# baldhat/yolov10-3D

Measured on AMD Instinct MI355X. Metric: train_images_per_sec, higher is better.
Workload: dtype bf16

## Files before the change

include/y3d.h:

```cpp
#ifndef Y3D_H
#define Y3D_H
#include <stdint.h>

#ifdef __cplusplus
extern "C" {
#endif

enum { Y3D_F32 = 0, Y3D_BF16 = 1 };
enum { Y3D_OK = 0, Y3D_ERR_INVALID = -1, Y3D_ERR_HIP = -2 };

const char* y3d_last_error(void);
int y3d_abi_version(void);
int y3d_device_info(char* name, int name_len, int* compute_units, int* lds_bytes, int* clock_khz);

int y3d_pack_weight_fwd(int dtype, const float* w_oihw, void* out, int Cout, int Cin_g, int Cin_g_pad, int kh, int kw, void* stream);
int y3d_pack_weight_dgrad(int dtype, const float* w_oihw, void* out, int Cout, int Cin_g, int groups, int kh, int kw, void* stream);
int y3d_mt_pack_weights(int dtype, const int64_t* desc, const int* chunk_tensor, const int* chunk_off, int nchunks, int chunk, void* stream);
int y3d_mt_fp8w_quantize(const int64_t* desc, const int* row_begin, int ntensors, int nrows, void* stream);
int y3d_fp8w_dequantize(const uint8_t* codes, const float* scale, float* w, int rows, int K, void* stream);
int y3d_fp8_quantize_act(const void* x, int64_t xsw, int64_t M, int C, uint8_t* q, uint8_t* s, void* stream);
int y3d_fp8_pack_weight_fwd(const uint8_t* codes, const float* scale, int rows, int Cg, uint8_t* wq, uint8_t* ws, void* stream);
int y3d_conv3x3_fp8_ok(int B, int H, int W, int Cin, int Cout, int groups);
int y3d_conv3x3_fp8_stat_rows(int B, int H, int W);
int y3d_fp8_scale_pitch(int C);
int y3d_conv3x3_fp8_fwd(const uint8_t* xq, const uint8_t* xs, int B, int H, int W, int Cin, const uint8_t* wq, const uint8_t* ws, void* y, int64_t ysw,
                        int Cout, int groups, float* stat_partials, const float* scale, const float* shift, int act, void* stream);
int y3d_fp8_quantize_grad(const void* dy, int64_t sw, const float* scale, int64_t M, int C, uint8_t* q, uint8_t* s, void* stream);
int y3d_fp8_pack_weight_dgrad(const uint8_t* codes, int Cout, int Cin, int groups, int lo, int hi, uint8_t* wq, uint8_t* ws, void* stream);
int y3d_conv3x3_fp8_dgrad_ok(int B, int H, int W, int Cin, int Cout, int groups);
int y3d_conv3x3_fp8_dgrad(const uint8_t* dyq, const uint8_t* dys, int64_t qsw, int spitch, int lo, int hi, int B, int H, int W, const uint8_t* wq, const uint8_t* ws,
                          void* dx, int64_t dxsw, int Cin, int groups, void* stream);
int y3d_conv_kpad(int dtype, int k_total);
int y3d_conv_stat_blocks(int B, int Ho, int Wo);
int y3d_conv2d_stat_rows(int dtype, int B, int H, int W, int Cin, int Cout, int groups, int kh, int kw, int stride, int pad);
enum { Y3D_OP_FWD = 0, Y3D_OP_BWD_DATA = 1, Y3D_OP_BWD_WEIGHT = 2 };
enum { Y3D_EPI_RAW = 0, Y3D_EPI_PARTIALS = 1, Y3D_EPI_AFFINE = 2, Y3D_EPI_AFFINE_RES = 3, Y3D_EPI_BIAS = 4 };
enum {
  Y3D_ROUTE_GENERIC = 0,
  Y3D_ROUTE_STREAM1X1 = 1,
  Y3D_ROUTE_SMALL = 2,
  Y3D_ROUTE_SMALL_S2 = 3,
  Y3D_ROUTE_S2_DGRAD = 4,
  Y3D_ROUTE_TILE8 = 5,
  Y3D_ROUTE_TILE16 = 6,
  Y3D_ROUTE_WIDE3_8 = 7,
  Y3D_ROUTE_WIDE3_16 = 8,
  Y3D_ROUTE_FLAT = 9,
  Y3D_ROUTE_WGRAD_SMALL = 10,
  Y3D_ROUTE_WGRAD_TILE = 11,
  Y3D_ROUTE_WGRAD_STREAM1X1 = 12
};
int y3d_conv2d_route(int dtype, int op, int epi, int B, int H, int W, int Cin, int Cout, int groups, int kh, int kw, int stride, int pad);
int y3d_conv2d_fwd(int dtype, const void* x, int64_t xsb, int64_t xsh, int64_t xsw, int B, int H, int W, int Cin,
                   const void* w_packed, const float* bias, void* y, int64_t ysw, int Ho, int Wo, int Cout, int groups,
                   int kh, int kw, int stride, int pad, float* stat_partials, void* stream);
int y3d_conv2d_fwd_affine(int dtype, const void* x, int64_t xsb, int64_t xsh, int64_t xsw, int B, int H, int W, int Cin,
                          const void* w_packed, const float* scale, const float* shift, int act, void* y, int64_t ysw, int Ho, int Wo,
                          int Cout, int groups, int kh, int kw, int stride, int pad, void* stream);
int y3d_conv2d_fwd_affine_res_ok(int dtype, int B, int H, int W, int Cin, int Cout, int groups, int kh, int kw, int stride, int pad);
int y3d_conv2d_fwd_affine_res(int dtype, const void* x, int64_t xsb, int64_t xsh, int64_t xsw, int B, int H, int W, int Cin,
                              const void* w_packed, const float* scale, const float* shift, int act, const void* res, int64_t rsw, void* y,
                              int64_t ysw, int Ho, int Wo, int Cout, int groups, int kh, int kw, int stride, int pad, void* stream);
int y3d_conv2d_bwd_data(int dtype, const void* dy, int64_t dsb, int64_t dsh, int64_t dsw, int B, int Ho, int Wo, int Cout,
                        const void* w_packed_dgrad, void* dx, int64_t xsw, int H, int W, int Cin, int groups, int kh, int kw,
                        int stride, int pad, void* stream);
int y3d_conv2d_wgrad_splits(int dtype, int B, int Ho, int Wo, int Cout, int Cin_g, int groups, int kh, int kw);
int y3d_conv2d_wgrad_plan(int dtype, int B, int H, int W, int Cin, int Cout, int groups, int kh, int kw, int stride, int pad);
int y3d_set_tile_kernels(int enable);
int y3d_set_stream1x1(int enable);
int y3d_get_stream1x1(void);
int y3d_get_tile_kernels(void);
int y3d_set_bn_wide_slabs(int enable);
int y3d_conv2d_bwd_weight(int dtype, const void* x, int64_t xsb, int64_t xsh, int64_t xsw, int B, int H, int W, int Cin,
                          int Cin_real, const void* dy, int64_t dsw, int Ho, int Wo, int Cout, int groups, int kh, int kw,
                          int stride, int pad, float* slab, int nsplit, float* grad_oihw, int accumulate, void* stream);

int y3d_dw_blocks(int64_t M);
int y3d_dw_wgrad_blocks(int64_t M);
int y3d_dw_pack_weight(const float* w_oihw, float* out_taps_c, int C, int kh, int kw, void* stream);
int y3d_dwconv2d_fwd(int dtype, const void* x, int64_t xsb, int64_t xsh, int64_t xsw, int B, int H, int W, int C,
                     const float* w_packed, void* y, int64_t ysw, int Ho, int Wo, int kh, int kw, int stride, int pad,
                     float* stat_partials, void* stream);
int y3d_dwconv2d_fwd_affine(int dtype, const void* x, int64_t xsb, int64_t xsh, int64_t xsw, int B, int H, int W, int C,
                            const float* w_packed, const float* scale, const float* shift, int act, int res_mode, const void* res, int64_t rsw,
                            void* z, int64_t zsw, int Ho, int Wo, int kh, int kw, int stride, int pad, void* stream);
int y3d_dwconv2d_bwd_data(int dtype, const void* dy, int64_t dsb, int64_t dsh, int64_t dsw, int B, int Ho, int Wo, int C,
                          const float* w_packed, void* dx, int64_t xsw, int H, int W, int kh, int kw, int stride, int pad,
                          void* stream);
int y3d_dwconv2d_bwd_weight(int dtype, const void* x, int64_t xsb, int64_t xsh, int64_t xsw, int B, int H, int W, int C,
                            const void* dy, int64_t dsw, int Ho, int Wo, int kh, int kw, int stride, int pad, float* slab,
                            float* grad_oihw, int accumulate, void* stream);

int y3d_bn_finalize(const float* partials, int nblk, int C, int64_t count, const float* gamma, const float* beta, float eps,
                    float momentum, float* running_mean, float* running_var, float* mean, float* invstd, float* scale,
                    float* shift, void* stream);
int y3d_bn_eval_scale(int C, const float* gamma, const float* beta, const float* running_mean, const float* running_var,
                      float eps, float* scale, float* shift, void* stream);
int y3d_bn_act_fwd(int dtype, const void* y, int64_t ysw, const float* scale, const float* shift, int act, int res_mode,
                   const void* res, int64_t rsw, void* z, int64_t zsw, int64_t P, int C, void* stream);
int y3d_bn_act_fwd_q(const void* y, int64_t ysw, const float* scale, const float* shift, int act, void* z, int64_t zsw, uint8_t* q, uint8_t* s,
                     int64_t P, int C, void* stream);
int y3d_bn_bwd_blocks(int64_t P, int C);
int y3d_bn_act_bwd_reduce(int dtype, const void* y, int64_t ysw, const void* dz, int64_t dsw, const void* res, int64_t rsw,
                          const float* scale, const float* shift, const float* mean, const float* invstd, int act,
                          int res_mode, float* partials, int64_t P, int C, void* stream);
int y3d_bn_bwd_finalize(const float* partials, int nblk, int C, int64_t count, float* dgamma, float* dbeta, int accumulate,
                        float* mean_g, float* mean_gx, void* stream);
int y3d_bn_act_bwd_apply(int dtype, const void* y, int64_t ysw, const void* dz, int64_t dsw, const void* res, int64_t rsw,
                         const float* scale, const float* shift, const float* mean, const float* invstd,
                         const float* mean_g, const float* mean_gx, int act, int res_mode, int train, void* dy, int64_t dysw,
                         void* dres, int64_t drsw, int64_t P, int C, void* stream);
int y3d_colsum_partials(int dtype, const void* x, int64_t xsw, float* partials, int64_t P, int C, void* stream);

int y3d_maxpool_fwd(int dtype, const void* x, int64_t xsb, int64_t xsh, int64_t xsw, void* y, int64_t ysw, uint8_t* argmax,
                    int B, int H, int W, int C, int k, void* stream);
int y3d_maxpool_bwd(int dtype, const void* dy, int64_t dsw, const uint8_t* argmax, void* dx, int64_t xsw, int B, int H, int W,
                    int C, int k, void* stream);
int y3d_upsample2x_fwd(int dtype, const void* x, int64_t xsb, int64_t xsh, int64_t xsw, void* y, int64_t ysw, int B, int H, int W,
                       int C, void* stream);
int y3d_upsample2x_bwd(int dtype, const void* dy, int64_t dsb, int64_t dsh, int64_t dsw, void* dx, int64_t xsw, int B, int H,
                       int W, int C, void* stream);
int y3d_copy2d(int dtype, const void* x, int64_t xsw, void* y, int64_t ysw, int64_t P, int C, void* stream);
int y3d_occupy_cus(int n, const int* flag, float* buf, int64_t nbuf, void* stream);
int y3d_add2d(int dtype, const void* a, int64_t asw, const void* b, int64_t bsw, void* y, int64_t ysw, int64_t P, int C, void* stream);
int y3d_nchw_to_nhwc(int dtype, const float* x_nchw, void* y_nhwc, int B, int C, int H, int W, int Cpad, void* stream);
int y3d_stem_im2col(int dtype, const float* x_nchw, void* out, int B, int H, int W, int Ho, int Wo, void* stream);
int y3d_stem_im2col_u8(int dtype, const uint8_t* x, int hwc, void* out, int B, int H, int W, int Ho, int Wo, void* stream);
int y3d_stem_conv_eval(const void* x, int in_mode, const float* wcol, const float* scale, const float* shift, int act, void* y, int64_t ysw,
                       int B, int H, int W, int Cout, void* stream);
int y3d_stem_conv_train_rows(int B, int H, int W);
int y3d_stem_conv_train(const void* x, int in_mode, const float* wcol, void* y, int64_t ysw, void* xcol, float* part, int B, int H, int W,
                        int Cout, void* stream);
int y3d_nhwc_to_nchw(int dtype, const void* x_nhwc, int64_t xsw, float* y_nchw, int B, int C, int H, int W, void* stream);
int y3d_proj_fwd(int dtype, const void* x, int64_t xsw, const float* w, const float* bias, void* y, int64_t ysw, int64_t P,
                 int Cin, int Cout, void* stream);
int y3d_proj_bwd_data(int dtype, const void* dy, int64_t dsw, const float* w, void* dx, int64_t xsw, int64_t P, int Cin, int Cout,
                      void* stream);
int y3d_proj_blocks(int64_t P);
int y3d_proj_bwd_weight(int dtype, const void* x, int64_t xsw, const void* dy, int64_t dsw, float* slab, float* bias_slab,
                        float* grad_w, float* grad_b, int accumulate, int64_t P, int Cin, int Cout, void* stream);
int y3d_slab_reduce(const float* slab, float* out, int nblk, int64_t n, int accumulate, void* stream);
int y3d_proj_group_fwd(int dtype, int nb, int cin, const void* x, int64_t xsw, const int* xoff, const float* const* w,
                       const float* const* b, const int* couts, void* y, int64_t ysw, int64_t P, void* stream);
int y3d_proj_group_bwd_data(int dtype, int nb, int cin, const void* dy, int64_t dsw, const int* xoff, const float* const* w,
                            const int* couts, void* dx, int64_t xsw, int64_t P, void* stream);
int y3d_proj_group_fwd_bn_mfma(int nb, int cin, const void* y_pre, int64_t ysw, const int* xoff, const float* const* w, const float* const* b,
                               const int* couts, const float* scale, const float* shift, int act, void* out, int64_t osw, int64_t P,
                               void* stream);
int y3d_proj_group_bwd_weight_bn_mfma_blocks(int64_t P);
int y3d_proj_group_bwd_weight_bn_mfma(int nb, int cin, const void* y_pre, int64_t ysw, const int* xoff, const void* dout, int64_t dsw,
                                      const int* couts, const float* scale, const float* shift, int act, float* slab, float* bslab,
                                      float* const* dw, float* const* db, int64_t P, void* stream);
int y3d_proj_group_bn_bwd_blocks(int64_t P);
int y3d_proj_group_bn_bwd(int mode, int nb, int cin, const void* y_pre, int64_t ysw, const int* xoff, const void* dout, int64_t dsw,
                          const float* const* w, const int* couts, const float* scale, const float* shift, const float* mean,
                          const float* invstd, const float* mean_g, const float* mean_gx, int act, float* partials, int nblk, void* dy,
                          int64_t dysw, int64_t P, int C, void* stream);
int y3d_proj_group_blocks(int64_t P);
int y3d_proj_group_fwd_bn(int dtype, int nb, int cin, const void* y_pre, int64_t xsw, const int* xoff, const float* const* w,
                          const float* const* b, const int* couts, const float* scale, const float* shift, int act, void* out,
                          int64_t ysw, int64_t P, void* stream);
int y3d_proj_group_bwd_weight_bn(int dtype, int nb, int cin, const void* y_pre, int64_t xsw, const int* xoff, const void* dy, int64_t dsw,
                                 const int* couts, const float* scale, const float* shift, int act, float* slab, float* bslab,
                                 float* const* dw, float* const* db, int64_t P, void* stream);
int y3d_proj_group_bwd_weight(int dtype, int nb, int cin, const void* x, int64_t xsw, const int* xoff, const void* dy, int64_t dsw,
                              const int* couts, float* slab, float* bslab, float* const* dw, float* const* db, int64_t P, void* stream);

int y3d_attn_fwd(int dtype, const void* qkv, int64_t qsw, void* out, int64_t osw, float* lse, int B, int N, int nh, int kd, int hd,
                 float scale, void* stream);
int y3d_attn_bwd(int dtype, const void* qkv, int64_t qsw, const void* out, int64_t osw, const void* dout, int64_t dsw,
                 const void* dv_extra, int64_t esw, const float* lse, float* delta, void* dqkv, int64_t gsw, int B, int N, int nh,
                 int kd, int hd, float scale, void* stream);

int y3d_tal3d_scratch_floats(int B, int n, int A, int topk);
int y3d_pad_targets(const float* rows, int nbox, int width, int B, int cap, float scale_x, float scale_y, float* out, int* n_used,
                    void* stream);
int y3d_tal3d_assign(int dtype, int nl, const void* const* maps, const int64_t* psw, const int* H, const int* W, const float* strides,
                     int B, int nc, const float* gt, int n, const float* calib, const float* mean_sizes, int topk, float alpha,
                     float beta, float gamma, int mode, float* scratch, uint8_t* fg_mask, int* target_gt_idx, float* target_scores, float* scal,
                     const int* n_used, void* stream);
int y3d_loss3d(int dtype, int nl, const void* const* maps, const int64_t* psw, void* const* grads, const int64_t* gsw, const int* H,
               const int* W, const float* strides, int B, int nc, const float* gt, int n, const uint8_t* fg_mask,
               const int* target_gt_idx, const float* target_scores, const float* scal, float w_loss2d, float w_cls, float w_depth,
               float w_offset3d, float w_size3d, float w_heading, float grad_scale, float* partials, float* items, void* stream);

int y3d_distill_loss(int dtype, int nl, const void* const* embs, const int64_t* psw, const int* H, const int* W, int B, int C,
                     const void* teacher, int teacher_dtype, int th, int tw, int64_t tsb, int64_t tsc, int64_t tsh, int64_t tsw,
                     const float* gt, int n, const uint8_t* fg_mask, const int* target_gt_idx, const float* scal, const uint8_t* mixed,
                     int img_w, int img_h, float T, float weight, int criterion, int no_mixup, int cap, int* counts, int* idx,
                     void* rows, float* partials, float* loss, void* stream);
int y3d_distill_scatter(int dtype, const void* rows, const int* idx, const int* nrows, const float* scale, int cap, int C, void* grad,
                        int64_t sb, int64_t sh, int64_t sw, int a0, int H, int W, void* stream);

int y3d_tal2d_assign(int dtype, int nl, const void* const* maps, const int64_t* psw, const int* H, const int* W, const float* strides,
                     int B, int nc, const float* gt, int n, int topk, float alpha, float beta, float* scratch, uint8_t* fg_mask,
                     int* target_gt_idx, float* target_scores, float* scal, const int* n_used, void* stream);
int y3d_loss2d(int dtype, int nl, const void* const* maps, const int64_t* psw, void* const* grads, const int64_t* gsw, const int* H,
               const int* W, const float* strides, int B, int nc, const float* gt, int n, const uint8_t* fg_mask,
               const int* target_gt_idx, const float* target_scores, const float* scal, float w_box, float w_cls, float w_dfl,
               float grad_scale, float* partials, float* items, void* stream);
int y3d_tal2d_scratch_floats(int B, int n, int A, int topk);
int y3d_tal2d_assign_crowded(int dtype, int nl, const void* const* maps, const int64_t* psw, const int* H, const int* W, const float* strides,
                             int B, int nc, const float* gt, int n, int topk, float alpha, float beta, float* scratch, uint8_t* fg_mask,
                             int* target_gt_idx, float* target_scores, float* scal, const int* n_used, void* stream);

int y3d_topk_cells(int dtype, const void* cls, int64_t psw, int B, int HW, int nc, int K, int* out_idx, void* stream);
int y3d_patch_gather(int dtype, const void* x, int64_t xsb, int64_t xsh, int64_t xsw, const int* idx, void* out, int B, int H, int W,
                     int C, int K, int ps, void* stream);
int y3d_head3d_scatter(int dtype, const void* cls, int64_t csw, const void* reg, int64_t rsw, const int* idx, void* map, int B, int HW,
                       int nc, int no, int K, void* stream);
int y3d_head3d_decode(int dtype, int nl, const void* const* maps, const int* H, const int* W, const float* strides, int B, int nc,
                      float* y, void* stream);
int y3d_head2d_decode(int dtype, int nl, const void* const* maps, const int* H, const int* W, const float* strides, int B, int nc,
                      float* y, void* stream);
int y3d_v10_postprocess_scratch_floats(int B, int A, int nc, int max_det);
int y3d_v10_postprocess(const float* y, int B, int C, int A, int nc, int max_det, int boxes_first, float* reg, float* scores,
                        int64_t* labels, float* scratch, void* stream);

int y3d_kitti_image_aug(const unsigned char* const* src, const unsigned char* const* src2, const int* hw, const int* flip, const double* trans_inv,
                        int B, int out_h, int out_w, int mode, void* out, void* stream);
int y3d_kde_depth_fusion(const float* predsO, int B, int K, const float* predsM, int KM, int C, float thres, float iou_thres, int nprop,
                         float* out, void* stream);
int y3d_kitti_decode(const float* preds, int B, int K, const double* calib, const double* ratio, const double* inv_trans,
                     const double* mean_size, int nc, int use_camera_dis, double threshold, double* out, unsigned char* keep, void* stream);
int y3d_kitti_encode_labels(const double* rec, const int* img_i, const double* img_f, int B, int out_w, int out_h, double min_depth,
                            double max_depth, int use_camera_dis, const double* mean_size, int n_cls, int max_objs, int64_t* cls,
                            double* bboxes, float* center_2d, float* size_2d, double* center_3d, double* size_3d, double* depth,
                            int64_t* heading_bin, double* heading_res, float* batch_idx, int* counts, double* calib, double* ratio_pad,
                            void* stream);
int y3d_json3d_encode_labels(const double* rec, const int* img_i, const double* img_f, int B, int dataset, int out_w, int out_h,
                             double min_depth, double max_depth, int use_camera_dis, const double* mean_size, int n_cls, int max_objs,
                             int64_t* cls, double* bboxes, float* center_2d, float* size_2d, double* center_3d, double* size_3d,
                             double* depth, int64_t* heading_bin, double* heading_res, float* batch_idx, int* counts, double* calib,
                             double* ratio_pad, void* stream);
int y3d_yolo2d_image_aug(const unsigned char* const* src, int n_src, const int* rec_i, const double* rec_f, const unsigned char* lut, int B,
                         int imgsz, int mode, void* out, void* stream);
int y3d_yolo2d_encode_labels(const float* rec, int n_rec, const int* lab_i, const float* lab_f, int B, int imgsz, int cap, float* cls,
                             float* bboxes, float* batch_idx, int* counts, void* stream);
int y3d_letterbox_image(const unsigned char* const* src_table, int n_src, const int* rec, int B, int H, int W, int mode, void* out,
                        void* stream);
int y3d_letterbox_labels(const float* rec, int n_rec, const int* lab_i, const float* lab_f, int B, int H, int W, int cap, float* cls,
                         float* bboxes, float* batch_idx, int* counts, void* stream);
int y3d_predict_rows(const float* preds, const float* meta, float conf, const int* classes, int n_cls, int B, int K, float* out, int* counts,
                     void* stream);
int y3d_predict3d_rows(const float* preds, int B, int K, const double* calib, const double* P2, const double* ratio,
                       const double* inv_trans, const double* mean_size, int nc, int use_camera_dis, double conf, const int* classes,
                       int n_cls, double* rows, double* corners3d, double* corners_img, int* counts, void* stream);

int y3d_kitti_eval_max_boxes(void);
int y3d_kitti_box_overlaps(int metric, const float* gt, const float* dt, const int* gt_off, const int* dt_off, const int64_t* ov_off,
                           int n_img, float* out, void* stream);
int y3d_kitti_eval_thresholds(const float* gt, const int* gt_code, const float* dt, const int* dt_code, const int* gt_off, const int* dt_off,
                              const int64_t* ov_off, const float* ov, int n_img, int total_gt, int metric, const int* cd, int ncd,
                              const double* min_ov, int nk, float* tp_score, int* nvalid, void* stream);
int y3d_kitti_eval_counts(const float* gt, const int* gt_code, const float* dt, const int* dt_code, const int* gt_off, const int* dt_off,
                          const int64_t* ov_off, const float* ov, int n_img, int metric, const int* cd, int ncd, const double* min_ov, int nk,
                          const float* thr, const int* nthr, int compute_aos, int* cnt, double* sim, double* pr, void* stream);

int y3d_det_metrics_max_gts(void);
int y3d_det_metrics_max_dets(void);
int y3d_box_iou(const float* box1, int n1, const float* box2, int n2, float eps, float* out, void* stream);
int y3d_match_predictions(const float* iou, const int* gt_cls, int n_gt, const int* det_cls, int n_det, const float* thr, int n_thr,
                          int* tp, void* stream);
int y3d_box_match_batch(int mode, const void* preds, const unsigned char* keep, int B, int K, const double* meta, int img_h, int img_w,
                        int single_cls, const float* gt_img, const float* gt_cls, const float* gt_box, int n_gt, const float* thr,
                        int n_thr, int* tp, double* conf, int* cls, int* status, void* stream);
int y3d_confusion_batch(int mode, const void* preds, const unsigned char* keep, int B, int K, const double* meta, int img_h, int img_w,
                        int single_cls, const float* gt_img, const float* gt_cls, const float* gt_box, int n_gt, int nc, double conf,
                        double iou_thres, int* matrix, int* status, void* stream);
int y3d_confusion_image(const float* gt_box, const int* gt_cls, int n_gt, const void* det, int det_f64, int n_det, int nc, double conf,
                        double iou_thres, int* matrix, int* status, void* stream);
int y3d_ap_per_class(const int* tp, const double* conf, const int* cls, int64_t n, const int* ucls, const double* nl, int nc, int n_thr,
                     const double* x_ap, int n_ap, const double* x_curve, int n_curve, double* ap, double* p_curve, double* r_curve,
                     void* stream);

int y3d_mt_sqnorm(const int64_t* grad_ptrs, const int64_t* sizes, const int* chunk_tensor, const int* chunk_off, int nchunks, int chunk,
                  float* partials, void* stream);
int y3d_mt_copy(const int64_t* src_ptrs, const int64_t* dst_ptrs, const int64_t* sizes, const int* chunk_tensor, const int* chunk_off,
                int nchunks, int chunk, float scale, void* stream);
int y3d_mt_clip_coef(const float* partials, int nchunks, float max_norm, float* out_norm_clip, void* stream);
int y3d_mt_sgd(const int64_t* param_ptrs, const int64_t* grad_ptrs, const int64_t* buf_ptrs, const int64_t* sizes, const float* lr,
               const float* wd, const int* chunk_tensor, const int* chunk_off, int nchunks, int chunk, float momentum, int nesterov,
               int first_step, const float* norm_clip, void* stream);

int y3d_mt_adamw(const int64_t* param_ptrs, const int64_t* grad_ptrs, const int64_t* m_ptrs, const int64_t* v_ptrs, const int64_t* sizes,
                 const float* lr, const float* wd, const int* chunk_tensor, const int* chunk_off, int nchunks, int chunk, float beta1, float beta2,
                 float eps, float bias_corr1, float bias_corr2_sqrt, const float* norm_clip, void* stream);
int y3d_mt_ema(const int64_t* ema_ptrs, const int64_t* model_ptrs, const int64_t* sizes, const int* reps, const int* chunk_tensor,
               const int* chunk_off, int nchunks, int chunk, float decay, float one_minus_decay, const float* guard, void* stream);

#ifdef __cplusplus
}
#endif
#endif
```

yolov10-3d_amd/_lib.py:

```python
from __future__ import annotations

import ctypes
import os
import re

_HERE = os.path.dirname(os.path.abspath(__file__))
LIB_PATH = os.path.join(_HERE, "liby3d_hip.so")
HEADER = os.path.join(os.path.dirname(_HERE), "include", "y3d.h")

F32, BF16 = 0, 1

_CT = {"int": ctypes.c_int, "int64_t": ctypes.c_int64, "float": ctypes.c_float, "double": ctypes.c_double}


class Y3DError(RuntimeError):
    pass


def parse_header(path: str = HEADER):
    src = open(path).read()
    src = re.sub(r"/\*.*?\*/", " ", src, flags=re.S)
    protos = {}
    for m in re.finditer(r"(const\s+char\s*\*|int)\s+(y3d_\w+)\s*\(([^;{]*?)\)\s*;", src, flags=re.S):
        ret, name, args = m.group(1), m.group(2), m.group(3).strip()
        argtypes = []
        if args and args != "void":
            for a in args.split(","):
                a = a.strip()
                if "*" in a:
                    argtypes.append(ctypes.c_void_p)
                else:
                    toks = a.split()
                    t = toks[1] if toks[0] == "const" else toks[0]
                    argtypes.append(_CT[t])
        protos[name] = (ctypes.c_char_p if "char" in ret else ctypes.c_int, argtypes)
    return protos


_PLAIN_INT = {"abi_version", "conv_kpad", "conv_stat_blocks", "conv2d_stat_rows", "conv2d_route", "conv2d_wgrad_splits", "conv2d_wgrad_plan", "set_tile_kernels", "set_stream1x1", "set_bn_wide_slabs", "get_stream1x1", "get_tile_kernels", "dw_blocks", "dw_wgrad_blocks", "bn_bwd_blocks", "proj_blocks", "proj_group_blocks", "proj_group_bn_bwd_blocks", "proj_group_bwd_weight_bn_mfma_blocks", "tal3d_scratch_floats", "tal2d_scratch_floats", "v10_postprocess_scratch_floats", "conv2d_fwd_affine_res_ok", "stem_conv_train_rows", "conv3x3_fp8_ok", "conv3x3_fp8_dgrad_ok", "conv3x3_fp8_stat_rows", "fp8_scale_pitch", "kitti_eval_max_boxes", "det_metrics_max_gts", "det_metrics_max_dets"}


class _Lib:
    def __init__(self):
        if not os.path.exists(LIB_PATH):
            raise Y3DError(
                f"{LIB_PATH} not found: build it with `python yolov10-3d_amd/csrc/build.py` "
                "(or __graft_entry__.build()). There is no CPU / PyTorch fallback for the HIP path.")
        self._dll = ctypes.CDLL(LIB_PATH)
        self.protos = parse_header()
        for name, (ret, argtypes) in self.protos.items():
            fn = getattr(self._dll, name)
            fn.restype = ret
            fn.argtypes = argtypes

    def last_error(self) -> str:
        return (self._dll.y3d_last_error() or b"").decode()

    def __getattr__(self, name):
        if name.startswith("_"):
            raise AttributeError(name)
        fn = getattr(self._dll, "y3d_" + name)
        ret = self.protos["y3d_" + name][0]
        if ret is not ctypes.c_int or name in _PLAIN_INT:
            setattr(self, name, fn)
            return fn

        def call(*a):
            rc = fn(*a)
            if rc != 0:
                raise Y3DError(f"y3d_{name} failed ({rc}): {self.last_error()}")
            return rc

        setattr(self, name, call)
        return call


_lib = None


def lib() -> _Lib:
    global _lib
    if _lib is None:
        _lib = _Lib()
    return _lib
```

yolov10-3d_amd/csrc/conv1x1_stream.hip:

```cpp
#include "common.h"
#include "conv_frag.h"
#include <cstdlib>

namespace {

struct PwP {
  const bf16_t* x;
  const bf16_t* w;
  const float *bias, *scale, *shift;
  bf16_t* y;
  float* part;
  long ysw;
  int xsw;
  int M, K, N, Kpad;
  int nkc, nmt, nnt, act;
  int G, PC;
  unsigned xbytes, ybytes, pbytes, wbytes;
};

template <int N> __device__ __forceinline__ void pw_wvm() { asm volatile("s_waitcnt vmcnt(%0)" ::"n"(N) : "memory"); }
__device__ __forceinline__ void pw_wvm_n(int n) {
#define PW_C(i) case i: pw_wvm<i>(); break;
#define PW_C8(i) PW_C(i) PW_C(i + 1) PW_C(i + 2) PW_C(i + 3) PW_C(i + 4) PW_C(i + 5) PW_C(i + 6) PW_C(i + 7)
  switch (n) {
    PW_C8(0) PW_C8(8) PW_C8(16) PW_C8(24) PW_C8(32) PW_C8(40) PW_C8(48) PW_C(56) PW_C(57) PW_C(58) PW_C(59) PW_C(60) PW_C(61) PW_C(62)
    default: pw_wvm<63>(); break;
  }
#undef PW_C8
#undef PW_C
}
typedef __attribute__((ext_vector_type(2))) unsigned pw_u32x2;

template <int BN, int WP, int WC, int NS, bool AFF, bool WRES>
__global__ __launch_bounds__(512) void conv1x1_stream_kernel(PwP p) {
  {
    const int g = blockIdx.y;
    p.x += (long)g * p.K;
    p.w += (long)g * p.N * p.Kpad;
    p.y += (long)g * p.N;
    if (p.bias) p.bias += g * p.N;
    if (p.scale) { p.scale += g * p.N; p.shift += g * p.N; }
    if (p.part) p.part += (long)g * p.N * 2;
  }
  constexpr int BM = 128;
  constexpr int TP = BM / WP / 16, TC = BN / WC / 16;
  static_assert(WP * WC == 8 && TP >= 1 && TC >= 1, "8 waves");
  constexpr int STAGE = BM * 128 + (WRES ? 0 : BN * 128);
  constexpr int ND = 2 + (WRES ? 0 : BN / 64);
  static_assert(WRES || BN % 64 == 0, "streamed weight tiles: whole DMA instructions per wave");
  extern __shared__ __attribute__((aligned(16))) char smem[];
  char* sW = smem;
  char* sA = smem + (WRES ? (size_t)p.nkc * BN * 128 : 0);
  const int tid = threadIdx.x, lane = tid & 63, wave = __builtin_amdgcn_readfirstlane(tid >> 6);
  const int wp = wave % WP, wc = wave / WP;
  const int bid = blockIdx.x, xcd = bid & 7, idx = bid >> 3;
  const int nt = idx % p.nnt, wk = (idx / p.nnt) * 8 + xcd, nwk = (gridDim.x / p.nnt);
  const int n0 = nt * BN;
  const int mine = wk < p.nmt ? (p.nmt - wk + nwk - 1) / nwk : 0;
  const int S = mine * p.nkc;
  if (S == 0) {
    if (p.part && tid < BN && n0 + tid < p.N) *(float2*)(p.part + ((long)wk * p.PC + n0 + tid) * 2) = make_float2(0.f, 0.f);
    return;
  }

  if (WRES)
  for (int i = tid; i < p.nkc * BN * 8; i += 512) {
    const int c = i & 7, r = (i >> 3) % BN, kc = i / (8 * BN);
    const int k = kc * 64 + c * 8, n = n0 + r;
    uint4 v = make_uint4(0, 0, 0, 0);
    if (n < p.N && k < p.Kpad) v = *(const uint4*)(p.w + (long)n * p.Kpad + k);
    *(uint4*)(sW + (kc * BN + r) * 128 + ((c ^ (r & 7)) << 4)) = v;
  }

  const __amdgpu_buffer_rsrc_t rx = __builtin_amdgcn_make_buffer_rsrc((void*)p.x, 0, (int)p.xbytes, 0x00020000);
  const __amdgpu_buffer_rsrc_t rw = __builtin_amdgcn_make_buffer_rsrc((void*)p.w, 0, (int)p.wbytes, 0x00020000);
  constexpr unsigned OOB = 0xfffffff0u;
  const int lrow = lane >> 3, lchunk = (lane & 7) ^ lrow;
  int is = 0, i_tile = wk, i_kc = 0, i_slot = 0;
  auto issue = [&]() {
    const bool live = is < S;
    const int k = i_kc * 64 + lchunk * 8;
#pragma unroll
    for (int h = 0; h < 2; ++h) {
      const int r = 16 * wave + 8 * h;
      const int m = i_tile * BM + r + lrow;
      const bool ok = live & (m < p.M) & (k < p.K);
      const unsigned off = (unsigned)(m * p.xsw + k) * 2u;
      __builtin_amdgcn_raw_ptr_buffer_load_lds(rx, (__attribute__((address_space(3))) void*)(sA + i_slot * STAGE + r * 128), 16, ok ? off : OOB, 0, 0, 0);
    }
    if (!WRES) {
#pragma unroll
      for (int h = 0; h < BN / 64; ++h) {
        const int r = (BN / 8) * wave + 8 * h;
        const int n = n0 + r + lrow;
        const bool ok = live & (n < p.N) & (k < p.K);
        __builtin_amdgcn_raw_ptr_buffer_load_lds(rw, (__attribute__((address_space(3))) void*)(sA + i_slot * STAGE + (BM + r) * 128), 16,
                                                 ok ? (unsigned)(n * p.Kpad + k) * 2u : OOB, 0, 0, 0);
      }
    }
    ++is;
    if (++i_kc == p.nkc) { i_kc = 0; i_tile += nwk; }
    if (++i_slot == NS) i_slot = 0;
  };
#pragma unroll
  for (int s = 0; s < NS - 1; ++s) issue();

  f32x4_t acc[TC][TP];
  const int lc = (lane >> 4) * 4, lp = lane & 15;
  int c_tile = wk, c_kc = 0, c_slot = 0;
  int hist[NS - 1];
#pragma unroll
  for (int i = 0; i < NS - 1; ++i) hist[i] = 0;
  const __amdgpu_buffer_rsrc_t ry = __builtin_amdgcn_make_buffer_rsrc((void*)p.y, 0, (int)p.ybytes, 0x00020000);
  asm volatile("s_waitcnt lgkmcnt(0)" ::: "memory");

  float ssum[TC][4], ssq[TC][4];
#pragma unroll
  for (int a = 0; a < TC; ++a)
#pragma unroll
    for (int j = 0; j < 4; ++j) { ssum[a][j] = 0.f; ssq[a][j] = 0.f; }

#pragma unroll 1
  for (int s = 0; s < S; ++s) {
    {
      int young = ND * (NS - 2);
#pragma unroll
      for (int i = 0; i < NS - 1; ++i) young += hist[i];
      pw_wvm_n(young);
#pragma unroll
      for (int i = 0; i < NS - 2; ++i) hist[i] = hist[i + 1];
      hist[NS - 2] = 0;
    }
    __builtin_amdgcn_s_barrier();
    issue();
    if (c_kc == 0) {
#pragma unroll
      for (int a = 0; a < TC; ++a)
#pragma unroll
        for (int b = 0; b < TP; ++b) acc[a][b] = (f32x4_t){0.f, 0.f, 0.f, 0.f};
    }
    const char* tA = sA + c_slot * STAGE + (wp * (BM / WP)) * 128;
    const char* tW = WRES ? sW + (c_kc * BN + wc * (BN / WC)) * 128 : sA + c_slot * STAGE + (BM + wc * (BN / WC)) * 128;
    const int nks = p.K - c_kc * 64 > 32 ? 2 : 1;
    for (int ks = 0; ks < nks; ++ks) {
      bf16x8_t fb[TP], fa[TC];
#pragma unroll
      for (int b = 0; b < TP; ++b) fb[b] = Frag<bf16_t>::load(tA, b * 16, ks, lane);
#pragma unroll
      for (int a = 0; a < TC; ++a) fa[a] = Frag<bf16_t>::load(tW, a * 16, ks, lane);
#pragma unroll
      for (int a = 0; a < TC; ++a)
#pragma unroll
        for (int b = 0; b < TP; ++b) acc[a][b] = __builtin_amdgcn_mfma_f32_16x16x32_bf16(fa[a], fb[b], acc[a][b], 0, 0, 0);
    }
    if (++c_slot == NS) c_slot = 0;
    if (++c_kc < p.nkc) continue;
    c_kc = 0;
#pragma unroll
    for (int a = 0; a < TC; ++a) {
      const int cl = wc * (BN / WC) + a * 16 + lc, co = n0 + cl;
      float bv[4] = {0.f, 0.f, 0.f, 0.f}, sv[4] = {1.f, 1.f, 1.f, 1.f}, hv[4] = {0.f, 0.f, 0.f, 0.f};
      if (AFF && p.bias) {
#pragma unroll
        for (int j = 0; j < 4; ++j) if (co + j < p.N) bv[j] = p.bias[co + j];
      }
      if (AFF && p.scale) {
#pragma unroll
        for (int j = 0; j < 4; ++j) if (co + j < p.N) { sv[j] = p.scale[co + j]; hv[j] = p.shift[co + j]; }
      }
#pragma unroll
      for (int b = 0; b < TP; ++b) {
        const int m = c_tile * BM + wp * (BM / WP) + b * 16 + lp;
        float v[4];
#pragma unroll
        for (int j = 0; j < 4; ++j) {
          float u = acc[a][b][j];
          if (AFF) {
            u += bv[j];
            if (p.scale) { u = u * sv[j] + hv[j]; if (p.act) u = silu_f(u); }
          }
          v[j] = bf2f(f2bf(u));
          ssum[a][j] += v[j];
          ssq[a][j] += v[j] * v[j];
        }
        const pw_u32x2 u = {(unsigned)f2bf(v[0]) | ((unsigned)f2bf(v[1]) << 16), (unsigned)f2bf(v[2]) | ((unsigned)f2bf(v[3]) << 16)};
        __builtin_amdgcn_raw_buffer_store_b64(u, ry, ((m < p.M) & (co < p.N)) ? (unsigned)(m * (int)p.ysw + co) * 2u : OOB, 0, 0);
      }
    }
    hist[NS - 2] += TC * TP;
    c_tile += nwk;
  }
  pw_wvm<0>();
  if (p.part) {
    __syncthreads();
    float* red = (float*)sA;
#pragma unroll
    for (int a = 0; a < TC; ++a)
#pragma unroll
      for (int j = 0; j < 4; ++j) {
        const float s = wave_xor_sum16(ssum[a][j]), q = wave_xor_sum16(ssq[a][j]);
        if (lp == 0) {
          const int cl = wc * (BN / WC) + a * 16 + lc + j;
          red[(wp * BN + cl) * 2] = s;
          red[(wp * BN + cl) * 2 + 1] = q;
        }
      }
    __syncthreads();
    if (tid < BN && n0 + tid < p.N) {
      float s = 0.f, q = 0.f;
#pragma unroll
      for (int w = 0; w < WP; ++w) { s += red[(w * BN + tid) * 2]; q += red[(w * BN + tid) * 2 + 1]; }
      float* dst = p.part + ((long)wk * p.PC + n0 + tid) * 2;
      dst[0] = s;
      dst[1] = q;
    }
  }
}

struct PwPlan {
  int bn, ns, nnt, grid, wres;
  size_t lds;
};

bool pw_plan(int M, int K, int N, PwPlan* pl, int G = 1) {
  const int nkc = cdiv(K, 64);
  const size_t cap = 160 * 1024;
  const int nmt = cdiv(M, 128);
  const int bns[4] = {256, 128, 64, 32};
  int bn = 0;
  for (int i = 0; i < 4; ++i) {
    const int b = bns[i];
    if (i < 3 && bns[i + 1] >= N) continue;
    if ((size_t)b * nkc * 128 + 3 * 16384 <= cap) { bn = b; break; }
  }
  const bool can_stream = N > 64 && nkc >= 2;
  bool wres = bn != 0 && (cdiv(N, bn) == 1 || (cdiv(N, bn) == 2 && nmt < 200));
  if (!wres && !can_stream) {
    if (!bn) return false;
    wres = true;
  }
  pl->wres = wres;
  if (wres) {
    const size_t wb = (size_t)bn * nkc * 128;
    pl->bn = bn;
    pl->ns = wb + 4 * 16384 <= cap ? 4 : 3;
    pl->lds = wb + pl->ns * 16384;
  } else {
    pl->bn = N > 128 ? 256 : 128;
    pl->ns = pl->bn == 256 ? 3 : 4;
    pl->lds = (size_t)pl->ns * (16384 + pl->bn * 128);
  }
  pl->nnt = cdiv(N, pl->bn);
  const int per_cu = pl->lds <= 80 * 1024 ? 2 : 1;
  int wpx = (32 * per_cu) / (pl->nnt * G);
  if (wpx < 1) wpx = 1;
  if (wpx > cdiv(nmt, 8)) wpx = cdiv(nmt, 8);
  pl->grid = 8 * wpx * pl->nnt;
  return true;
}

template <int BN, int WP, int WC, int NS, bool AFF, bool WRES>
void pw_launch_1(const PwP& p, const PwPlan& pl, hipStream_t st) {
  static bool attr = false;
  if (!attr) {
    (void)hipFuncSetAttribute((const void*)conv1x1_stream_kernel<BN, WP, WC, NS, AFF, WRES>, hipFuncAttributeMaxDynamicSharedMemorySize, 160 * 1024);
    attr = true;
  }
  hipLaunchKernelGGL((conv1x1_stream_kernel<BN, WP, WC, NS, AFF, WRES>), dim3(pl.grid, p.G), dim3(512), pl.lds, st, p);
}

template <int BN, int WP, int WC>
void pw_launch_ns(const PwP& p, const PwPlan& pl, hipStream_t st) {
  const bool aff = p.bias || p.scale;
  if (pl.ns == 4) { if (aff) pw_launch_1<BN, WP, WC, 4, true, true>(p, pl, st); else pw_launch_1<BN, WP, WC, 4, false, true>(p, pl, st); }
  else { if (aff) pw_launch_1<BN, WP, WC, 3, true, true>(p, pl, st); else pw_launch_1<BN, WP, WC, 3, false, true>(p, pl, st); }
}

}

static int g_stream1x1 = 1;

extern "C" int y3d_get_stream1x1(void) { return g_stream1x1; }

extern "C" int y3d_set_stream1x1(int enable) {
  const int old = g_stream1x1;
  g_stream1x1 = enable ? 1 : 0;
  return old;
}

int y3d_conv1x1_stream_ok(int dtype, long M, int K, int N, long xsw, int G) {
  if (!g_stream1x1 || dtype != Y3D_BF16 || K % 8 != 0 || K < 32 || N < 8 || N % 4 != 0 || M < 128 || G < 1 || G > 64) return 0;
  if ((M * xsw + (long)G * K) * 2 >= (1L << 32) - 64 || M * N * G * 2 >= (1L << 31)) return 0;
  PwPlan pl;
  if (!pw_plan((int)M, K, N, &pl, G)) return 0;
  return 1;
}

int y3d_conv1x1_stream_rows(long M, int K, int N, int G) {
  PwPlan pl;
  if (!pw_plan((int)M, K, N, &pl, G)) return 0;
  return pl.grid / pl.nnt;
}

int y3d_conv1x1_stream_launch(const void* x, long xsw, const void* w, int Kpad, const float* bias, const float* scale, const float* shift, int act,
                              void* y, long ysw, float* part, long M, int K, int N, int G, void* stream) {
  PwPlan pl;
  Y3D_CHECK(pw_plan((int)M, K, N, &pl, G), "conv1x1_stream: no tile plan for K=%d N=%d", K, N);
  Y3D_CHECK(((uintptr_t)x & 15) == 0 && xsw % 8 == 0 && ((uintptr_t)w & 15) == 0 && Kpad % 8 == 0 && ((uintptr_t)y & 7) == 0 && ysw % 4 == 0,
            "conv1x1_stream: operand alignment");
  PwP p;
  p.x = (const bf16_t*)x; p.w = (const bf16_t*)w; p.bias = bias; p.scale = scale; p.shift = shift; p.y = (bf16_t*)y; p.part = part;
  p.ysw = ysw; p.xsw = (int)xsw; p.M = (int)M; p.K = K; p.N = N; p.Kpad = Kpad;
  p.nkc = cdiv(K, 64); p.nmt = cdiv(M, 128); p.nnt = pl.nnt; p.act = act; p.G = G; p.PC = G * N;
  p.xbytes = (unsigned)(((M - 1) * xsw + K) * 2);
  Y3D_CHECK(((M - 1) * ysw + (long)G * N) * 2 < (1L << 32) - 64 && M * ysw < (1L << 31), "conv1x1_stream: output tensor beyond 32-bit byte offsets");
  p.ybytes = (unsigned)(((M - 1) * ysw + N) * 2);
  p.pbytes = part ? (unsigned)((long)p.nmt * N * 8) : 0u;
  hipStream_t st = (hipStream_t)stream;
  p.wbytes = (unsigned)((long)N * Kpad * 2);
  if (!pl.wres) {
    const bool aff = bias || scale;
    if (pl.bn == 256) { if (aff) pw_launch_1<256, 2, 4, 3, true, false>(p, pl, st); else pw_launch_1<256, 2, 4, 3, false, false>(p, pl, st); }
    else { if (aff) pw_launch_1<128, 4, 2, 4, true, false>(p, pl, st); else pw_launch_1<128, 4, 2, 4, false, false>(p, pl, st); }
    Y3D_LAUNCH_CHECK();
    return Y3D_OK;
  }
  switch (pl.bn) {
    case 256: pw_launch_ns<256, 2, 4>(p, pl, st); break;
    case 128: pw_launch_ns<128, 4, 2>(p, pl, st); break;
    case 64: pw_launch_ns<64, 8, 1>(p, pl, st); break;
    default: pw_launch_ns<32, 8, 1>(p, pl, st); break;
  }
  Y3D_LAUNCH_CHECK();
  return Y3D_OK;
}
```

Measured before the change: 1468.

## Add small-M streamed 1x1 conv path with 128-wide streamed weight tiles

Generalizes the streamed 1x1 conv kernel body over block M and wave count, then adds a small-problem variant. It uses BN=128 streamed weight tiles, two pipeline stages and a smaller LDS footprint. The planner sends ungrouped convs with moderate M and N of at least 128 to this variant when the resident-weight plan would launch few blocks, aiming to raise occupancy and parallelism. The trade-off is that weights are re-streamed per M tile instead of held resident, and the shallower pipeline may expose more memory latency.

```diff
diff --git a/include/y3d.h b/include/y3d.h
--- a/include/y3d.h
+++ b/include/y3d.h
@@ -69,6 +69,8 @@
 int y3d_set_tile_kernels(int enable);
 int y3d_set_stream1x1(int enable);
 int y3d_get_stream1x1(void);
+int y3d_set_stream1x1_small(int enable);
+int y3d_conv1x1_stream_plan_kind(int64_t M, int K, int N, int G);
 int y3d_get_tile_kernels(void);
 int y3d_set_bn_wide_slabs(int enable);
 int y3d_conv2d_bwd_weight(int dtype, const void* x, int64_t xsb, int64_t xsh, int64_t xsw, int B, int H, int W, int Cin,
diff --git a/yolov10-3d_amd/_lib.py b/yolov10-3d_amd/_lib.py
--- a/yolov10-3d_amd/_lib.py
+++ b/yolov10-3d_amd/_lib.py
@@ -37,7 +37,7 @@
     return protos
 
 
-_PLAIN_INT = {"abi_version", "conv_kpad", "conv_stat_blocks", "conv2d_stat_rows", "conv2d_route", "conv2d_wgrad_splits", "conv2d_wgrad_plan", "set_tile_kernels", "set_stream1x1", "set_bn_wide_slabs", "get_stream1x1", "get_tile_kernels", "dw_blocks", "dw_wgrad_blocks", "bn_bwd_blocks", "proj_blocks", "proj_group_blocks", "proj_group_bn_bwd_blocks", "proj_group_bwd_weight_bn_mfma_blocks", "tal3d_scratch_floats", "tal2d_scratch_floats", "v10_postprocess_scratch_floats", "conv2d_fwd_affine_res_ok", "stem_conv_train_rows", "conv3x3_fp8_ok", "conv3x3_fp8_dgrad_ok", "conv3x3_fp8_stat_rows", "fp8_scale_pitch", "kitti_eval_max_boxes", "det_metrics_max_gts", "det_metrics_max_dets"}
+_PLAIN_INT = {"abi_version", "conv_kpad", "conv_stat_blocks", "conv2d_stat_rows", "conv2d_route", "conv2d_wgrad_splits", "conv2d_wgrad_plan", "set_tile_kernels", "set_stream1x1", "set_stream1x1_small", "conv1x1_stream_plan_kind", "set_bn_wide_slabs", "get_stream1x1", "get_tile_kernels", "dw_blocks", "dw_wgrad_blocks", "bn_bwd_blocks", "proj_blocks", "proj_group_blocks", "proj_group_bn_bwd_blocks", "proj_group_bwd_weight_bn_mfma_blocks", "tal3d_scratch_floats", "tal2d_scratch_floats", "v10_postprocess_scratch_floats", "conv2d_fwd_affine_res_ok", "stem_conv_train_rows", "conv3x3_fp8_ok", "conv3x3_fp8_dgrad_ok", "conv3x3_fp8_stat_rows", "fp8_scale_pitch", "kitti_eval_max_boxes", "det_metrics_max_gts", "det_metrics_max_dets"}
 
 
 class _Lib:
diff --git a/yolov10-3d_amd/csrc/conv1x1_stream.hip b/yolov10-3d_amd/csrc/conv1x1_stream.hip
--- a/yolov10-3d_amd/csrc/conv1x1_stream.hip
+++ b/yolov10-3d_amd/csrc/conv1x1_stream.hip
@@ -31,8 +31,8 @@
 }
 typedef __attribute__((ext_vector_type(2))) unsigned pw_u32x2;
 
-template <int BN, int WP, int WC, int NS, bool AFF, bool WRES>
-__global__ __launch_bounds__(512) void conv1x1_stream_kernel(PwP p) {
+template <int BM, int BN, int WP, int WC, int NS, bool AFF, bool WRES>
+__device__ __forceinline__ void pw_body(PwP p) {
   {
     const int g = blockIdx.y;
     p.x += (long)g * p.K;
@@ -42,12 +42,13 @@
     if (p.scale) { p.scale += g * p.N; p.shift += g * p.N; }
     if (p.part) p.part += (long)g * p.N * 2;
   }
-  constexpr int BM = 128;
+  constexpr int NW = WP * WC, NT = NW * 64;
   constexpr int TP = BM / WP / 16, TC = BN / WC / 16;
-  static_assert(WP * WC == 8 && TP >= 1 && TC >= 1, "8 waves");
+  static_assert((NW == 8 || NW == 4) && TP >= 1 && TC >= 1 && BN <= NT, "4 or 8 waves; one thread per channel in the folds");
   constexpr int STAGE = BM * 128 + (WRES ? 0 : BN * 128);
-  constexpr int ND = 2 + (WRES ? 0 : BN / 64);
-  static_assert(WRES || BN % 64 == 0, "streamed weight tiles: whole DMA instructions per wave");
+  constexpr int PD = BM / (8 * NW), WD = BN / (8 * NW);
+  constexpr int ND = PD + (WRES ? 0 : WD);
+  static_assert(BM % (8 * NW) == 0 && (WRES || BN % (8 * NW) == 0), "whole DMA instructions per wave");
   extern __shared__ __attribute__((aligned(16))) char smem[];
   char* sW = smem;
   char* sA = smem + (WRES ? (size_t)p.nkc * BN * 128 : 0);
@@ -64,7 +65,7 @@
   }
 
   if (WRES)
-  for (int i = tid; i < p.nkc * BN * 8; i += 512) {
+  for (int i = tid; i < p.nkc * BN * 8; i += NT) {
     const int c = i & 7, r = (i >> 3) % BN, kc = i / (8 * BN);
     const int k = kc * 64 + c * 8, n = n0 + r;
     uint4 v = make_uint4(0, 0, 0, 0);
@@ -81,8 +82,8 @@
     const bool live = is < S;
     const int k = i_kc * 64 + lchunk * 8;
 #pragma unroll
-    for (int h = 0; h < 2; ++h) {
-      const int r = 16 * wave + 8 * h;
+    for (int h = 0; h < PD; ++h) {
+      const int r = 8 * PD * wave + 8 * h;
       const int m = i_tile * BM + r + lrow;
       const bool ok = live & (m < p.M) & (k < p.K);
       const unsigned off = (unsigned)(m * p.xsw + k) * 2u;
@@ -90,8 +91,8 @@
     }
     if (!WRES) {
 #pragma unroll
-      for (int h = 0; h < BN / 64; ++h) {
-        const int r = (BN / 8) * wave + 8 * h;
+      for (int h = 0; h < WD; ++h) {
+        const int r = 8 * WD * wave + 8 * h;
         const int n = n0 + r + lrow;
         const bool ok = live & (n < p.N) & (k < p.K);
         __builtin_amdgcn_raw_ptr_buffer_load_lds(rw, (__attribute__((address_space(3))) void*)(sA + i_slot * STAGE + (BM + r) * 128), 16,
@@ -217,12 +218,22 @@
   }
 }
 
+template <int BN, int WP, int WC, int NS, bool AFF, bool WRES>
+__global__ __launch_bounds__(512) void conv1x1_stream_kernel(PwP p) { pw_body<128, BN, WP, WC, NS, AFF, WRES>(p); }
+
+template <int WP, bool AFF>
+__global__ __launch_bounds__(512) void conv1x1_stream_small_kernel(PwP p) { pw_body<128, 128, WP, 8 / WP, 2, AFF, false>(p); }
+
 struct PwPlan {
   int bn, ns, nnt, grid, wres;
   size_t lds;
+  int kind, wp;
 };
 
+int g_stream1x1_small = 1;
+
 bool pw_plan(int M, int K, int N, PwPlan* pl, int G = 1) {
+  pl->kind = 0;
   const int nkc = cdiv(K, 64);
   const size_t cap = 160 * 1024;
   const int nmt = cdiv(M, 128);
@@ -256,6 +267,17 @@
   if (wpx < 1) wpx = 1;
   if (wpx > cdiv(nmt, 8)) wpx = cdiv(nmt, 8);
   pl->grid = 8 * wpx * pl->nnt;
+  pl->wp = pl->bn == 256 ? 2 : 4;
+  if (g_stream1x1_small && G == 1 && can_stream && pl->bn >= 128 && nmt <= 400 && (!wres || pl->grid < 256)) {
+    const int workers = pl->grid / pl->nnt;
+    pl->kind = 1;
+    pl->wres = 0;
+    pl->bn = 128;
+    pl->ns = 2;
+    pl->lds = 2 * (128 * 128 + 128 * 128);
+    pl->nnt = cdiv(N, 128);
+    pl->grid = workers * pl->nnt;
+  }
   return true;
 }
 
@@ -269,6 +291,16 @@
   hipLaunchKernelGGL((conv1x1_stream_kernel<BN, WP, WC, NS, AFF, WRES>), dim3(pl.grid, p.G), dim3(512), pl.lds, st, p);
 }
 
+template <int WP, bool AFF>
+void pw_launch_small(const PwP& p, const PwPlan& pl, hipStream_t st) {
+  static bool attr = false;
+  if (!attr) {
+    (void)hipFuncSetAttribute((const void*)conv1x1_stream_small_kernel<WP, AFF>, hipFuncAttributeMaxDynamicSharedMemorySize, 160 * 1024);
+    attr = true;
+  }
+  hipLaunchKernelGGL((conv1x1_stream_small_kernel<WP, AFF>), dim3(pl.grid, 1), dim3(512), pl.lds, st, p);
+}
+
 template <int BN, int WP, int WC>
 void pw_launch_ns(const PwP& p, const PwPlan& pl, hipStream_t st) {
   const bool aff = p.bias || p.scale;
@@ -286,6 +318,18 @@
   const int old = g_stream1x1;
   g_stream1x1 = enable ? 1 : 0;
   return old;
+}
+
+extern "C" int y3d_set_stream1x1_small(int enable) {
+  const int old = g_stream1x1_small;
+  g_stream1x1_small = enable ? 1 : 0;
+  return old;
+}
+
+extern "C" int y3d_conv1x1_stream_plan_kind(int64_t M, int K, int N, int G) {
+  PwPlan pl;
+  if (M < 128 || M >= (1L << 31) || !pw_plan((int)M, K, N, &pl, G)) return 0;
+  return pl.kind;
 }
 
 int y3d_conv1x1_stream_ok(int dtype, long M, int K, int N, long xsw, int G) {
@@ -318,6 +362,14 @@
   p.pbytes = part ? (unsigned)((long)p.nmt * N * 8) : 0u;
   hipStream_t st = (hipStream_t)stream;
   p.wbytes = (unsigned)((long)N * Kpad * 2);
+  if (pl.kind == 1) {
+    const bool aff = bias || scale;
+    if (aff) pw_launch_small<2, true>(p, pl, st);
+    else if (pl.wp == 2) pw_launch_small<2, false>(p, pl, st);
+    else pw_launch_small<4, false>(p, pl, st);
+    Y3D_LAUNCH_CHECK();
+    return Y3D_OK;
+  }
   if (!pl.wres) {
     const bool aff = bias || scale;
     if (pl.bn == 256) { if (aff) pw_launch_1<256, 2, 4, 3, true, false>(p, pl, st); else pw_launch_1<256, 2, 4, 3, false, false>(p, pl, st); }
```

Result: no change. 1475, median of 6 (+0.5%).
